# bernardo-torres/1d-spectral-optimal-transport

Hardware: AMD Instinct MI355X
Metric: sot_loss_evals_per_sec (higher is better)
Workload: dtype f32

## Files before the change

1d-spectral-optimal-transport_amd/csrc/sot_full_common.hpp:

```cpp
#pragma once
#include "sot_launch.hpp"

namespace sot {

#ifdef SOT_STAMPS
#define SOT_PH(sacc, i) do { if ((sacc) != nullptr) { __builtin_amdgcn_sched_barrier(0); const unsigned long long now_ = __builtin_readcyclecounter(); \
                              (sacc)[i] += now_ - (sacc)[15]; (sacc)[15] = now_; __builtin_amdgcn_sched_barrier(0); } } while (0)
#else
#define SOT_PH(sacc, i) do { } while (0)
#endif

template <int NSTEPS>
__device__ __forceinline__ float mass_column_nx(const float* part, int c)
{
    constexpr int NFULL = NSTEPS >> 4;
    constexpr int NREAD = NFULL + ((NSTEPS & 15) ? 1 : 0);
    float pre[NREAD];
#pragma unroll
    for (int h = 0; h < NREAD; ++h) pre[h] = part[(h << 5) + c];
    float a0 = 0.0f, a1 = 0.0f, a2 = 0.0f, a3 = 0.0f;
#pragma unroll
    for (int h = 0; h < NFULL; ++h) {
        a0 = pre[h];
        a1 += a0; a0 = 0.0f;
        if ((((h + 1) << 4) & (15 << 4)) == 0) {
            a2 += a1; a1 = 0.0f;
            if ((((h + 1) << 4) & (15 << 8)) == 0) { a3 += a2; a2 = 0.0f; }
        }
    }
    if (NSTEPS & 15) a0 = pre[NFULL];
    return ((a0 + a1) + a2) + a3;
}

__host__ __device__ constexpr int staged_index(int e, bool swz) { return swz ? (e ^ (((e >> 5) & 1) << 2)) : e; }

template <bool SQ, int N, bool SWZ>
__device__ __forceinline__ float mass_fold_nx(const float* raw, const float* colbuf)
{
    const float4* c4 = reinterpret_cast<const float4*>(colbuf);
    const float4 a0 = c4[0], a1 = c4[1], b0 = c4[2], b1 = c4[3], c0 = c4[4], c1 = c4[5], d0 = c4[6], d1 = c4[7];
    const float p0 = ((a0.x + b0.x) + c0.x) + d0.x, p1 = ((a0.y + b0.y) + c0.y) + d0.y;
    const float p2 = ((a0.z + b0.z) + c0.z) + d0.z, p3 = ((a0.w + b0.w) + c0.w) + d0.w;
    const float p4 = ((a1.x + b1.x) + c1.x) + d1.x, p5 = ((a1.y + b1.y) + c1.y) + d1.y;
    const float p6 = ((a1.z + b1.z) + c1.z) + d1.z, p7 = ((a1.w + b1.w) + c1.w) + d1.w;
    float fin = 0.0f;
#pragma unroll
    for (int k = (N >> 3) << 3; k < N; ++k) { const float w = raw[staged_index(k, SWZ)]; fin += SQ ? w * w : w; }
    fin += p0; fin += p1; fin += p2; fin += p3; fin += p4; fin += p5; fin += p6; fin += p7;
    return fin;
}

#define SOT_FULL_WALK_UNROLL 32

template <int NU, int NV>
__device__ __forceinline__ uint32_t merge_path_fixed32(uint32_t ub1, uint32_t vd1, int D)
{
    constexpr int TOPK = merge_steps_top(NU < NV ? NU : NV);
    const int lo = max(0, D - NV), hi = min(D, NU);
    uint32_t posb = ub1 + 4u * (uint32_t)lo;
    const uint32_t hib = ub1 + 4u * (uint32_t)hi;
#pragma unroll
    for (int k = TOPK; k >= -1; --k) {
        const uint32_t step4 = 4u * (uint32_t)(k >= 1 ? (1 << k) + 1 : (k == 0 ? 2 : 1));
        const uint32_t candb = posb + step4;
        const float u = lds_load(candb);
        const float v = lds_load(vd1 - candb);
        const int take = (int)(candb <= hib) & (int)(u <= v);
        posb = take ? candb : posb;
    }
    return posb;
}

template <int G, int CPT, int N>
__device__ __forceinline__ void fetch_row_dwords(const float* __restrict__ x, const float* __restrict__ y, int t, float (&rx)[CPT],
                                                 float (&ry)[CPT])
{
#pragma unroll
    for (int k = 0; k < CPT; ++k) {
        if (k * G < N) {
            const int e = t + k * G;
            const bool ok = ((k + 1) * G <= N) || (e < N);
            rx[k] = ok ? x[e] : 0.0f;
            ry[k] = ok ? y[e] : 0.0f;
        }
    }
}

typedef __amdgpu_buffer_rsrc_t RowBuffer;
__device__ __forceinline__ RowBuffer row_buffer(const float* row, int n)
{
    return __builtin_amdgcn_make_buffer_rsrc(const_cast<float*>(row), (short)0, n * 4, 0x00020000);
}
__device__ __forceinline__ float row_buffer_load(RowBuffer rb, int element)
{
    return __builtin_bit_cast(float, __builtin_amdgcn_raw_buffer_load_b32(rb, element * 4, 0, 0));
}
__device__ __forceinline__ void row_buffer_store(RowBuffer rb, int element, float v)
{
    __builtin_amdgcn_raw_buffer_store_b32(__builtin_bit_cast(unsigned int, v), rb, element * 4, 0, 0);
}

template <int G, int CPT>
__device__ __forceinline__ void fetch_row_dwords_rt(const float* __restrict__ x, const float* __restrict__ y, int t, int n, float (&rx)[CPT],
                                                    float (&ry)[CPT])
{
    const RowBuffer bx = row_buffer(x, n), by = row_buffer(y, n);
#pragma unroll
    for (int k = 0; k < CPT; ++k) {
        rx[k] = row_buffer_load(bx, t + k * G);
        ry[k] = row_buffer_load(by, t + k * G);
    }
}

template <int G, int CPT, int NX>
__device__ __forceinline__ void fetch_row(const float* __restrict__ x, const float* __restrict__ y, int t, int n, float (&rx)[CPT], float (&ry)[CPT]);

template <int G, int CPT>
__device__ __forceinline__ void fetch_full_row(const float* __restrict__ x, const float* __restrict__ y, int t, float (&rx)[CPT],
                                               float (&ry)[CPT])
{
    const float4* x4 = reinterpret_cast<const float4*>(x);
    const float4* y4 = reinterpret_cast<const float4*>(y);
#pragma unroll
    for (int k = 0; k < CPT / 4; ++k) {
        const float4 vx = x4[t + k * G], vy = y4[t + k * G];
        rx[4 * k] = vx.x; rx[4 * k + 1] = vx.y; rx[4 * k + 2] = vx.z; rx[4 * k + 3] = vx.w;
        ry[4 * k] = vy.x; ry[4 * k + 1] = vy.y; ry[4 * k + 2] = vy.z; ry[4 * k + 3] = vy.w;
    }
}

template <int G, int CPT>
__device__ __forceinline__ void fetch_row_columns(const float* __restrict__ x, const float* __restrict__ y, int t, float (&rx)[CPT], float (&ry)[CPT])
{
    static_assert(CPT == 8, "16 steps per task: two registers arrays of 8");
    const bool isy = t >= G / 2;
    const int task = isy ? t - G / 2 : t;
    const float* const src = (isy ? y : x) + ((task >> 5) << 9) + (task & 31);
#pragma unroll
    for (int k = 0; k < 8; ++k) { rx[k] = src[k << 5]; ry[k] = src[(8 + k) << 5]; }
}

template <int G, int CPT, int N>
struct ColumnsNX {
    static constexpr int NSTEPS = N >> 5, NCH = (NSTEPS + 15) >> 4, NT = 32 * NCH, CHUNK = NSTEPS < 16 ? NSTEPS : 16;
    static constexpr int TPT = (2 * NT) / G;
    static constexpr int NV = TPT * CHUNK;
    static constexpr int MIN_BINS = 1025;
    static constexpr bool OK = (2 * NT) % G == 0 && TPT >= 1 && NV + 1 <= 2 * CPT && (N & 7) == 1 && N >= MIN_BINS;
};
template <int CPT>
__device__ __forceinline__ float& column_slot(float (&rx)[CPT], float (&ry)[CPT], int j) { return j < CPT ? rx[j] : ry[j - CPT]; }

template <int G, int CPT, int N>
__device__ __forceinline__ void fetch_row_columns_nx(const float* __restrict__ x, const float* __restrict__ y, int t, float (&rx)[CPT], float (&ry)[CPT])
{
    using C = ColumnsNX<G, CPT, N>;
#pragma unroll
    for (int i = 0; i < C::TPT; ++i) {
        const int id = t + i * G;
        const bool isy = id >= C::NT;
        const int task = isy ? id - C::NT : id;
        const float* const src = (isy ? y : x) + ((task >> 5) << 9) + (task & 31);
#pragma unroll
        for (int k = 0; k < C::CHUNK; ++k) column_slot<CPT>(rx, ry, i * C::CHUNK + k) = src[k << 5];
    }
    float tail = 0.0f;
    if (t < 2) tail = (t ? y : x)[N - 1];
    column_slot<CPT>(rx, ry, C::NV) = tail;
}

template <int G, int CPT, int NX>
__device__ __forceinline__ void fetch_row(const float* __restrict__ x, const float* __restrict__ y, int t, int n, float (&rx)[CPT], float (&ry)[CPT])
{
    if constexpr (NX == 0) fetch_row_columns<G, CPT>(x, y, t, rx, ry);
    else if constexpr (NX > 0 && ColumnsNX<G, CPT, (NX > 0 ? NX : 129)>::OK) fetch_row_columns_nx<G, CPT, NX>(x, y, t, rx, ry);
    else if constexpr (NX == 0) fetch_full_row<G, CPT>(x, y, t, rx, ry);
    else if constexpr (NX > 0) fetch_row_dwords<G, CPT, NX>(x, y, t, rx, ry);
    else fetch_row_dwords_rt<G, CPT>(x, y, t, n, rx, ry);
}

struct FullLayout {
    int padcap;
    int nU, nV;
    int part;
    int colbuf;
    int wtot;
    int red;
    int grad;
    int goff;
    int rowf;
    int posf;
    int total;
};

template <int G, int CPT, int ROWS, int GRAD = 0, int NX = 0>
__host__ __device__ constexpr FullLayout full_layout()
{
    constexpr int CAP = G * CPT, N = NX > 0 ? NX : CAP, NW = G / kWave, NT = 32 * (((N >> 5) + 15) >> 4);
    FullLayout L{};
    L.padcap = align4(merge_steps(2 * N, G)) + 4;
    L.nU = L.padcap + CAP + 4;
    L.nV = CAP + 4;
    L.part = L.nU + L.nV;
    L.colbuf = L.part + 2 * NT;
    L.wtot = L.colbuf + 64;
    L.red = L.wtot + 4 * NW;
    L.grad = align4(L.red + NW + 4);
    L.goff = GRAD == 2 ? L.grad - L.nU : L.grad;
    L.rowf = GRAD == 2 ? L.grad + L.nV : GRAD ? L.grad + L.nU + L.nV : L.grad;
    L.posf = L.nU + L.nV;
    L.total = ROWS * L.rowf + L.posf;
    return L;
}

template <int G, int CPT, int ROWS, int GRAD, int NX = 0>
struct FullGeo {
    static_assert(ROWS >= 1 && ROWS <= 4, "row groups per workgroup");
    static constexpr int CAP = G * CPT;
    static constexpr bool RT = NX < 0;
    static constexpr int N = NX > 0 ? NX : CAP;
    static constexpr bool ALIGNED = (NX == 0);
    static constexpr int NSTEPS = N >> 5;
    static_assert(N <= CAP && N >= 64 && CPT >= 2 && CPT <= 17, "the row fits its geometry");
    static_assert(!ALIGNED || CPT == 8, "rows that fill their geometry: 8 contiguous elements (two 16-B halves) per thread");
    static constexpr bool SWZ = CPT == 8 && !RT;
    static_assert(NX <= 0 || CAP - N >= 1, "NX is for rows shorter than the capacity");
    static_assert(RT || NSTEPS < 16 || NSTEPS % 16 == 0, "every column is either one partial chunk or whole 16-step chunks");
    static_assert(RT || (N >> 3) == NSTEPS * 4, "no left-over 8-lane vectors (N mod 32 < 8)");
    static_assert(!SWZ || ((N >> 5) & 1) == 0 || (N & 7) == 0, "the scalar tail sits in an unswapped staging block");
    static_assert(((G >> 5) & 1) == 0, "the staging swizzle of element t + k*G must not depend on k");
    static constexpr int BLOCK = ROWS * G;
    static constexpr int NW = G / kWave;
    static constexpr int K = 2 * N;
    static constexpr int E = merge_steps(K, G);
    static constexpr int GA = (K + E - 1) / E;
    static constexpr int PAD = GA * E - K;
    static constexpr int NCH = (NSTEPS + 15) >> 4;
    static constexpr int CHUNK = NSTEPS < 16 ? NSTEPS : 16;
    static constexpr int NT = 32 * NCH;
    static constexpr FullLayout L = full_layout<G, CPT, ROWS, GRAD, NX>();
    static_assert(PAD + 1 <= L.padcap, "room for the virtual predecessor in front of the padding");
};

struct FullCtx {
    float* U; float* V; float* part; float* colbuf; double* wtot; float* red; float* Sv;
    const float* Uw;
    const float* PX; const float* PY;
    int rg, t, lane, wv;
    bool dn, x_ident, y_ident;
};

template <int G, int CPT, int ROWS, int GRAD, int NX = 0, bool RP = false>
__device__ __forceinline__ FullCtx full_setup(const FwdArgs& a, float* smem)
{
    using Geo = FullGeo<G, CPT, ROWS, GRAD, NX>;
    constexpr FullLayout L = Geo::L;
    constexpr int N = Geo::N, PAD = Geo::PAD;
    FullCtx c;
    const int tid = threadIdx.x;
    c.rg = __builtin_amdgcn_readfirstlane(tid / G);
    c.t = tid - c.rg * G;
    c.lane = tid & (kWave - 1);
    c.wv = __builtin_amdgcn_readfirstlane(c.t >> 6);
    c.dn = a.flags & SOT_FLAG_DONT_NORMALIZE;
    float* const base = smem + c.rg * L.rowf;
    c.U = base + L.padcap;
    c.V = base + L.nU;
    c.part = base + L.part;
    c.colbuf = base + L.colbuf;
    c.wtot = reinterpret_cast<double*>(base + L.wtot);
    c.red = base + L.red;
    c.Sv = c.red + Geo::NW;
    c.Uw = c.U - PAD;
    c.x_ident = true; c.y_ident = true;
    if (a.ident != nullptr) { c.x_ident = a.ident[0] != 0; c.y_ident = a.ident[1] != 0; }
    float* const PX = smem + ROWS * L.rowf + L.padcap;
    float* const PY = smem + ROWS * L.rowf + L.nU;
    c.PX = PX; c.PY = PY;
    const int nlast = (Geo::RT ? a.n : N) - 1;
    if (!RP) {
#pragma unroll
        for (int e = tid; e < N; e += Geo::BLOCK) {
            const int es = Geo::RT ? min(e, nlast) : e;
            PX[e] = a.xpos[es]; PY[e] = a.ypos[es];
        }
        if (tid < PAD) PX[tid - PAD] = a.xpos[0];
        if (tid == 0) {
            PX[N] = a.xpos[nlast];
            PY[N] = a.ypos[nlast];
        }
    }
    if (c.t < PAD) c.U[c.t - PAD] = 0.0f;
    for (int e = N + 1 + c.t; e < Geo::CAP; e += G) { c.U[e] = 0.0f; c.V[e] = 0.0f; }
    if (c.t == 0) {
        c.U[N] = INFINITY; c.V[N] = INFINITY;
        c.U[-PAD - 1] = -INFINITY; c.V[-1] = -INFINITY;
        if (Geo::RT) { c.U[N + 1] = 0.0f; c.V[N + 1] = 0.0f; }
    }
    return c;
}

template <int G, int CPT, int ROWS, int GRAD, bool SQ, int NX = 0, bool TO_LDS = true, bool RAW_OUT = (GRAD != 0)>
__device__ __forceinline__ void full_build_cdfs(const FwdArgs& a, const FullCtx& c, float (&rx)[CPT], float (&ry)[CPT],
                                                const float* nxt_x, const float* nxt_y, float (&wx)[CPT], float (&wy)[CPT],
                                                float& Sx, float& Sy, float (&cu)[CPT], float (&cv)[CPT], unsigned long long* sacc = nullptr,
                                                const int* psx = nullptr, const int* psy = nullptr)
{
    (void)sacc;
    using Geo = FullGeo<G, CPT, ROWS, GRAD, NX>;
    constexpr int N = Geo::N, NW = Geo::NW, NT = Geo::NT, CHUNK = Geo::CHUNK;
    constexpr bool ALIGNED = Geo::ALIGNED, RT = Geo::RT;
    float* const U = c.U; float* const V = c.V; float* const part = c.part; float* const colbuf = c.colbuf;
    double* const wtot = c.wtot; float* const Sv = c.Sv;
    const int t = c.t, lane = c.lane, wv = c.wv;
    const bool dn = c.dn, x_ident = c.x_ident, y_ident = c.y_ident;
    constexpr bool SWZ = Geo::SWZ;
    static_assert(G % 16 == 0, "whole 16-lane groups per row");
    const int q0s = SWZ ? (t ^ ((t >> 3) & 1)) : t;
    const int ownf = SWZ ? ((t >> 2) & 1) : 0;
    constexpr bool COLUMNS_NX = (NX > 0) && ColumnsNX<G, CPT, (NX > 0 ? NX : 129)>::OK;
    constexpr bool COLUMNS = ALIGNED || COLUMNS_NX;
    constexpr bool PRESQ = COLUMNS && SQ && !RAW_OUT;
    if constexpr (COLUMNS_NX) {
        using C = ColumnsNX<G, CPT, (NX > 0 ? NX : 129)>;
        static_assert(!COLUMNS_NX || (C::NT == NT && C::CHUNK == CHUNK && !SWZ), "the task layout of the chunk sums below");
#pragma unroll
        for (int i = 0; i < C::TPT; ++i) {
            const int id = t + i * G;
            const bool isy = id >= NT;
            const int task = isy ? id - NT : id;
            float* const dst = (isy ? V : U) + ((task >> 5) << 9) + (task & 31);
            float v[C::CHUNK];
#pragma unroll
            for (int k = 0; k < C::CHUNK; ++k) { const float w = column_slot<CPT>(rx, ry, i * C::CHUNK + k); v[k] = PRESQ ? w * w : w; }
#pragma unroll
            for (int k = 0; k < C::CHUNK; ++k) dst[k << 5] = v[k];
            if (!(isy && dn)) {
                float acc = 0.0f;
#pragma unroll
                for (int k = 0; k < C::CHUNK; ++k) acc += (SQ && !PRESQ) ? v[k] * v[k] : v[k];
                part[id] = acc;
            }
        }
        if (t < 2) { const float w = column_slot<CPT>(rx, ry, C::NV); (t ? V : U)[N - 1] = PRESQ ? w * w : w; }
    } else if constexpr (COLUMNS) {
        static_assert(2 * NT == G, "one (column, chunk) task per thread");
        const bool isy = t >= NT;
        const int task = isy ? t - NT : t;
        float* const dst = (isy ? V : U) + ((task >> 5) << 9) + (task & 31);
        float* const dsto = (isy ? V : U) + ((task >> 5) << 9) + ((task & 31) ^ (SWZ ? 4 : 0));
        float v[16];
#pragma unroll
        for (int k = 0; k < 8; ++k) { v[k] = PRESQ ? rx[k] * rx[k] : rx[k]; v[8 + k] = PRESQ ? ry[k] * ry[k] : ry[k]; }
#pragma unroll
        for (int k = 0; k < 16; ++k) ((k & 1) ? dsto : dst)[k << 5] = v[k];
        if (!(isy && dn)) {
            float acc = 0.0f;
#pragma unroll
            for (int k = 0; k < 16; ++k) acc += (SQ && !PRESQ) ? v[k] * v[k] : v[k];
            part[t] = acc;
        }
    } else if constexpr (ALIGNED) {
#pragma unroll
        for (int k = 0; k < CPT / 4; ++k) {
            reinterpret_cast<float4*>(U)[q0s + k * G] = make_float4(rx[4 * k], rx[4 * k + 1], rx[4 * k + 2], rx[4 * k + 3]);
            reinterpret_cast<float4*>(V)[q0s + k * G] = make_float4(ry[4 * k], ry[4 * k + 1], ry[4 * k + 2], ry[4 * k + 3]);
        }
    } else {
        const int es = SWZ ? (t ^ (((t >> 5) & 1) << 2)) : t;
#pragma unroll
        for (int k = 0; k < CPT; ++k) {
            if (RT || (k * G < N && (((k + 1) * G <= N) || (t + k * G < N)))) { U[es + k * G] = rx[k]; V[es + k * G] = ry[k]; }
        }
    }
    SOT_PH(sacc, 1);
    row_sync<NW>();
    SOT_PH(sacc, 2);

    const MassPlan mp = make_mass_plan(RT ? a.n : N);
    if constexpr (COLUMNS) {
    } else if constexpr (RT) {
        mass_chunk_sums<G, SQ>(U, part, mp, t);
        if (!dn) mass_chunk_sums<G, SQ>(V, part + NT, mp, t);
    } else {
#pragma unroll
    for (int id0 = 0; id0 < 2 * NT; id0 += G) {
        const int id = id0 + t;
        const bool isy = id >= NT;
        if (id < 2 * NT && !(isy && dn)) {
            const int task = isy ? id - NT : id;
            const float* src = (isy ? V : U) + ((task >> 5) << 9) + (task & 31);
            const float* srco = (isy ? V : U) + ((task >> 5) << 9) + ((task & 31) ^ (SWZ ? 4 : 0));
            float v[CHUNK];
#pragma unroll
            for (int s2 = 0; s2 < CHUNK; ++s2) { const float w = ((s2 & 1) ? srco : src)[s2 << 5]; v[s2] = SQ ? w * w : w; }
            float acc = 0.0f;
#pragma unroll
            for (int s2 = 0; s2 < CHUNK; ++s2) acc += v[s2];
            part[id] = acc;
        }
    }
    }
    SOT_PH(sacc, 3);
    if constexpr (!COLUMNS) row_sync<NW>();
    SOT_PH(sacc, 4);
    __builtin_amdgcn_s_setprio(kMassPrio);
    if (NW >= 2) {
        if (wv < 2 && !(wv == 1 && dn)) {
            const float* raw = wv ? V : U;
            float* cb = colbuf + 32 * wv;
            if (lane < 32) {
                if constexpr (RT) cb[lane] = mass_column<SQ>(raw, part + wv * NT, mp, lane);
                else cb[lane] = mass_column_nx<Geo::NSTEPS>(part + wv * NT, lane);
            }
            __builtin_amdgcn_fence(__ATOMIC_RELEASE, "wavefront");
            __builtin_amdgcn_wave_barrier();
            __builtin_amdgcn_fence(__ATOMIC_ACQUIRE, "wavefront");
            float S;
            if constexpr (RT) S = mass_fold<SQ>(raw, cb, mp.n);
            else S = mass_fold_nx<(SQ && !PRESQ), N, SWZ>(raw, cb);
            if (lane == 0) { Sv[wv] = S; Sv[2 + wv] = 1.0f / guard_mass(S); }
        }
    } else {
        const int half = lane >> 5, col = lane & 31;
        const bool use_y = half && !dn;
        float* cb = colbuf + 32 * half;
        if constexpr (RT) cb[col] = mass_column<SQ>(use_y ? V : U, part + (use_y ? NT : 0), mp, col);
        else cb[col] = mass_column_nx<Geo::NSTEPS>(part + (use_y ? NT : 0), col);
        __builtin_amdgcn_fence(__ATOMIC_RELEASE, "wavefront");
        __builtin_amdgcn_wave_barrier();
        __builtin_amdgcn_fence(__ATOMIC_ACQUIRE, "wavefront");
        float S;
        if constexpr (RT) S = mass_fold<SQ>(use_y ? V : U, cb, mp.n);
        else S = mass_fold_nx<(SQ && !PRESQ), N, SWZ>(use_y ? V : U, cb);
        if (col == 0) { Sv[half] = S; Sv[2 + half] = 1.0f / guard_mass(S); }
    }
    __builtin_amdgcn_s_setprio(0);
    const int e0 = t * CPT;
    const int h0 = e0 + 4 * ownf, h1 = e0 + 4 * (1 - ownf);
    if (x_ident) {
        if constexpr (CPT == 8) {
            const float4 v0 = *reinterpret_cast<const float4*>(U + h0), v1 = *reinterpret_cast<const float4*>(U + h1);
            wx[0] = v0.x; wx[1] = v0.y; wx[2] = v0.z; wx[3] = v0.w; wx[4] = v1.x; wx[5] = v1.y; wx[6] = v1.z; wx[7] = v1.w;
        } else {
#pragma unroll
            for (int k = 0; k < CPT; ++k) wx[k] = U[e0 + k];
        }
    } else if (psx != nullptr) {
#pragma unroll
        for (int k = 0; k < CPT; ++k) wx[k] = U[psx[k]];
    } else {
#pragma unroll
        for (int k = 0; k < CPT; ++k) {
            const int sx = (e0 + k < (RT ? a.n : N)) ? a.xperm[e0 + k] : N + 1;
            wx[k] = U[SWZ ? (sx ^ (((sx >> 5) & 1) << 2)) : sx];
        }
    }
    if (y_ident) {
        if constexpr (CPT == 8) {
            const float4 v0 = *reinterpret_cast<const float4*>(V + h0), v1 = *reinterpret_cast<const float4*>(V + h1);
            wy[0] = v0.x; wy[1] = v0.y; wy[2] = v0.z; wy[3] = v0.w; wy[4] = v1.x; wy[5] = v1.y; wy[6] = v1.z; wy[7] = v1.w;
        } else {
#pragma unroll
            for (int k = 0; k < CPT; ++k) wy[k] = V[e0 + k];
        }
    } else if (psy != nullptr) {
#pragma unroll
        for (int k = 0; k < CPT; ++k) wy[k] = V[psy[k]];
    } else {
#pragma unroll
        for (int k = 0; k < CPT; ++k) {
            const int sy = (e0 + k < (RT ? a.n : N)) ? a.yperm[e0 + k] : N + 1;
            wy[k] = V[SWZ ? (sy ^ (((sy >> 5) & 1) << 2)) : sy];
        }
    }
    if ((N < Geo::CAP || RT) && e0 + CPT > (RT ? a.n : N)) {
#pragma unroll
        for (int k = 0; k < CPT; ++k) {
            if (e0 + k >= (RT ? a.n : N)) { wx[k] = 0.0f; wy[k] = 0.0f; }
        }
    }
    SOT_PH(sacc, 5);
    row_sync<NW>();
    SOT_PH(sacc, 6);

    Sx = Sv[0]; Sy = dn ? Sx : Sv[1];
    const float rSx = Sv[2], rSy = dn ? rSx : Sv[3];
    const float Sxh = guard_mass(Sx), Syh = guard_mass(Sy);
    double px[CPT], py[CPT];
    double runx = 0.0, runy = 0.0;
    {
        float qx[CPT], qy[CPT];
        uint32_t risk = 0xFFFFFFFFu;
#pragma unroll
        for (int k = 0; k < CPT; ++k) {
            qx[k] = div_by_row_constant((SQ && !PRESQ) ? wx[k] * wx[k] : wx[k], Sxh, rSx, risk);
            qy[k] = div_by_row_constant((SQ && !PRESQ) ? wy[k] * wy[k] : wy[k], Syh, rSy, risk);
        }
        const bool slow = (risk < kFastDivMinBits) || !(Sxh <= 0x1p40f) || !(Syh <= 0x1p40f);
        if (__builtin_amdgcn_ballot_w64(slow) != 0ull) {
            asm volatile("; IEEE division fallback" ::: "memory");
#pragma unroll
            for (int k = 0; k < CPT; ++k) {
                qx[k] = ((SQ && !PRESQ) ? wx[k] * wx[k] : wx[k]) / Sxh;
                qy[k] = ((SQ && !PRESQ) ? wy[k] * wy[k] : wy[k]) / Syh;
            }
        }
#pragma unroll
        for (int k = 0; k < CPT; ++k) {
            runx += (double)qx[k]; runy += (double)qy[k];
            px[k] = runx; py[k] = runy;
        }
    }
    const double inx = wave_incl_scan(runx), iny = wave_incl_scan(runy);
    double exx = wave_shift_right1(inx), exy = wave_shift_right1(iny);
    if (NW > 1 && lane == kWave - 1) { wtot[wv] = inx; wtot[NW + wv] = iny; }
    SOT_PH(sacc, 7);
    row_sync<NW>();
    SOT_PH(sacc, 8);
    if constexpr (NW > 1) {
        double ox = 0.0, oy = 0.0;
        for (int w = 0; w < wv; ++w) { ox += wtot[w]; oy += wtot[NW + w]; }
        exx += ox; exy += oy;
    }
#pragma unroll
    for (int k = 0; k < CPT; ++k) { cu[k] = (float)(exx + px[k]); cv[k] = (float)(exy + py[k]); }
    if constexpr (TO_LDS) {
        if (CPT % 4 == 0 && (N == Geo::CAP || e0 + CPT <= N)) {
#pragma unroll
            for (int k = 0; k + 3 < CPT; k += 4) {
                *reinterpret_cast<float4*>(U + e0 + k) = make_float4(cu[k], cu[k + 1], cu[k + 2], cu[k + 3]);
                *reinterpret_cast<float4*>(V + e0 + k) = make_float4(cv[k], cv[k + 1], cv[k + 2], cv[k + 3]);
            }
        } else {
#pragma unroll
            for (int k = 0; k < CPT; ++k) {
                if (e0 + k < N) { U[e0 + k] = cu[k]; V[e0 + k] = cv[k]; }
            }
        }
    }
    if (nxt_x != nullptr) fetch_row<G, CPT, NX>(nxt_x, nxt_y, t, a.n, rx, ry);
    if constexpr (TO_LDS) row_sync<NW>();
}

template <int G, int CPT, int ROWS, int GRAD, int NX>
__device__ __forceinline__ void rowpos_row_setup(const FwdArgs& a, const FullCtx& c, int64_t rowc, int (&ix)[CPT], int (&iy)[CPT], int (&psx)[CPT], int (&psy)[CPT])
{
    using Geo = FullGeo<G, CPT, ROWS, GRAD, NX>;
    constexpr int N = Geo::N, NW = Geo::NW, PAD = Geo::PAD;
    static_assert(ROWS == 1 && NX == 0 && CPT == 8, "per-row positions: one row per workgroup, rows that fill the 8-element geometry");
    const int t = c.t;
    const uint16_t* const pr = a.perm_in + rowc * (2 * (int64_t)N);
    const float* const xp = a.xpos + rowc * a.xps;
    const float* const yp = a.ypos + rowc * a.yps;
    const uint4 qx = *reinterpret_cast<const uint4*>(pr + t * CPT), qy = *reinterpret_cast<const uint4*>(pr + N + t * CPT);
    float vx[CPT], vy[CPT];
#pragma unroll
    for (int k = 0; k < CPT; ++k) { vx[k] = xp[t + k * G]; vy[k] = yp[t + k * G]; }
    const uint32_t wqx[4] = {qx.x, qx.y, qx.z, qx.w}, wqy[4] = {qy.x, qy.y, qy.z, qy.w};
#pragma unroll
    for (int k = 0; k < CPT; ++k) {
        ix[k] = (int)((wqx[k >> 1] >> (16 * (k & 1))) & (uint32_t)(N - 1));
        iy[k] = (int)((wqy[k >> 1] >> (16 * (k & 1))) & (uint32_t)(N - 1));
        psx[k] = Geo::SWZ ? (ix[k] ^ (((ix[k] >> 5) & 1) << 2)) : ix[k];
        psy[k] = Geo::SWZ ? (iy[k] ^ (((iy[k] >> 5) & 1) << 2)) : iy[k];
    }
    float* const Um = c.U; float* const Vm = c.V;
#pragma unroll
    for (int k = 0; k < CPT; ++k) { Um[t + k * G] = vx[k]; Vm[t + k * G] = vy[k]; }
    row_sync<NW>();
    float gx[CPT], gy[CPT];
#pragma unroll
    for (int k = 0; k < CPT; ++k) { gx[k] = Um[ix[k]]; gy[k] = Vm[iy[k]]; }
    float* const PXw = const_cast<float*>(c.PX); float* const PYw = const_cast<float*>(c.PY);
    *reinterpret_cast<float4*>(PXw + t * CPT) = make_float4(gx[0], gx[1], gx[2], gx[3]);
    *reinterpret_cast<float4*>(PXw + t * CPT + 4) = make_float4(gx[4], gx[5], gx[6], gx[7]);
    *reinterpret_cast<float4*>(PYw + t * CPT) = make_float4(gy[0], gy[1], gy[2], gy[3]);
    *reinterpret_cast<float4*>(PYw + t * CPT + 4) = make_float4(gy[4], gy[5], gy[6], gy[7]);
    if (t < PAD) PXw[t - PAD] = gx[0];
    if (t == G - 1) { PXw[N] = gx[CPT - 1]; PYw[N] = gy[CPT - 1]; }
    row_sync<NW>();
}

}
```

1d-spectral-optimal-transport_amd/csrc/sot_full_fwd.hpp:

```cpp
#pragma once
#include "sot_full_common.hpp"

namespace sot {

constexpr int kFwd17MinWaves = 1;

constexpr int kFwd1025OneWaveRows = 6144;
constexpr int kRt1024OneWaveRows = 8192;

template <int E, int PM, bool LIM, uint32_t POFF4>
__device__ __forceinline__ float merge_walk_full(uint32_t ou, uint32_t ov, bool first, float p)
{
    float w = lds_load(ou), wp = lds_load(ou + POFF4);
    float r = lds_load(ov), rp = lds_load(ov + POFF4);
    float qprev = fmaxf(lds_load(ou - 4u), lds_load(ov - 4u));
    if (first) qprev = 0.0f;
    uint32_t pw = ou + 4u, pr = ov + 4u;
    float acc = 0.0f;
#pragma unroll SOT_FULL_WALK_UNROLL
    for (int s2 = 0; s2 < E; ++s2) {
        const bool c = w <= r;
        const float q = c ? w : r;
        const float cost = transport_cost<PM>(wp, rp, p);
        float delta = q - qprev;
        if (LIM && q > 1.0f) delta = 0.0f;
        acc = fmaf(delta, cost, acc);
        qprev = q;
        const uint32_t nx = c ? pw : pr;
        pr = c ? pr : pw;
        pw = nx + 4u;
        r = c ? r : w;
        rp = c ? rp : wp;
        w = lds_load(nx);
        wp = lds_load(nx + POFF4);
    }
    return acc;
}

template <int G, int CPT, int ROWS, int NX>
__device__ __forceinline__ void owner_perm_slots(const FwdArgs& a, const int* perm, int t, int (&ps)[CPT])
{
    using Geo = FullGeo<G, CPT, ROWS, false, NX>;
    constexpr int N = Geo::N;
    const int nreal = Geo::RT ? a.n : N;
#pragma unroll
    for (int k = 0; k < CPT; ++k) {
        const int sx = (t * CPT + k < nreal) ? perm[t * CPT + k] : N + 1;
        ps[k] = Geo::SWZ ? (sx ^ (((sx >> 5) & 1) << 2)) : sx;
    }
}

constexpr int kFwdMinWaves = 1;
constexpr int kRt512MinWaves = 4;

template <int G, int CPT, int ROWS, int PM, bool LIM, bool SQ, int NX = 0, bool RP = false>
__global__ __launch_bounds__(ROWS * G, (G == 512 && NX < 0) ? kRt512MinWaves : (CPT == 17) ? kFwd17MinWaves : kFwdMinWaves) void sot_forward_full_kernel(const FwdArgs a)
{
    static_assert(!RP || (ROWS == 1 && NX == 0 && CPT == 8), "per-row positions: one row per workgroup, rows that fill the 8-element geometry");
    using Geo = FullGeo<G, CPT, ROWS, false, NX>;
    constexpr FullLayout L = Geo::L;
    constexpr int N = Geo::N, NW = Geo::NW, E = Geo::E, GA = Geo::GA, PAD = Geo::PAD;
    extern __shared__ __attribute__((aligned(16))) float smem[];
    const int64_t row_step = (int64_t)gridDim.x * ROWS;
    int64_t row0 = (int64_t)blockIdx.x * ROWS;
    float rx[CPT], ry[CPT];
    FullCtx cm = full_setup<G, CPT, ROWS, false, NX, RP>(a, smem);
    if constexpr (RP) { cm.x_ident = false; cm.y_ident = false; }
    const FullCtx c = cm;
    if constexpr (NW == 1) __syncthreads();
    const int rg = c.rg, t = c.t, lane = c.lane, wv = c.wv;
    float* const V = c.V; float* const red = c.red;
    const float* const Uw = c.Uw;
    if (row0 < a.B) {
        const int64_t r = min(row0 + rg, a.B - 1);
        fetch_row<G, CPT, NX>(a.x + r * a.xs, a.y + r * a.ys, t, a.n, rx, ry);
    }

#ifdef SOT_STAMPS
    unsigned long long sbuf[16] = {};
    unsigned long long* const sacc = (threadIdx.x == 0 && blockIdx.x == gridDim.x / 2) ? sbuf : nullptr;
#else
    constexpr unsigned long long* sacc = nullptr;
#endif
    constexpr bool HOIST_PERM = CPT <= 9;
    int psx[HOIST_PERM ? CPT : 1] = {}, psy[HOIST_PERM ? CPT : 1] = {};
    if constexpr (HOIST_PERM && !RP) {
        if (!c.x_ident) owner_perm_slots<G, CPT, ROWS, NX>(a, a.xperm, t, psx);
        if (!c.y_ident) owner_perm_slots<G, CPT, ROWS, NX>(a, a.yperm, t, psy);
    }
    for (; row0 < a.B; row0 += row_step) {
        const int64_t row = row0 + rg;
        const bool valid = row < a.B;
        const bool more = row0 + row_step < a.B;
        const int64_t rn = min(row0 + row_step + rg, a.B - 1);
        float wx[CPT], wy[CPT], cu[CPT], cv[CPT];
        float Sx, Sy;
#ifdef SOT_STAMPS
        if (sacc != nullptr) sacc[15] = __builtin_readcyclecounter();
#endif
        if constexpr (RP) {
            int ix[CPT], iy[CPT];
            rowpos_row_setup<G, CPT, ROWS, false, NX>(a, c, min(row, a.B - 1), ix, iy, psx, psy);
        }
        full_build_cdfs<G, CPT, ROWS, false, SQ, NX>(a, c, rx, ry, more ? a.x + rn * a.xs : nullptr,
                                                     more ? a.y + rn * a.ys : nullptr, wx, wy, Sx, Sy, cu, cv, sacc, HOIST_PERM ? psx : nullptr,
                                                     HOIST_PERM ? psy : nullptr);
        SOT_PH(sacc, 9);

        float acc = 0.0f;
        __builtin_amdgcn_s_setprio(kWalkPrio);
        if (GA == G || t < GA) {
            constexpr int VOFF = L.nU - L.padcap + PAD;
            const int D0 = t * E;
            (void)VOFF;
            const uint32_t ub1 = lds_addr(Uw) - 4u;
            const uint32_t vd1 = lds_addr(V) + 4u * (uint32_t)D0 + ub1;
            const uint32_t pb = merge_path_fixed32<N + PAD, N>(ub1, vd1, D0);
            SOT_PH(sacc, 10);
            const uint32_t ou = pb + 4u;
            const uint32_t ov = vd1 - pb;
            constexpr uint32_t ROWB = 4u * (uint32_t)L.rowf;
            if (ROWS == 1 || rg == ROWS - 1) acc = merge_walk_full<E, PM, LIM, ROWB>(ou, ov, D0 == 0, a.p);
            else if (ROWS == 2 || rg == ROWS - 2) acc = merge_walk_full<E, PM, LIM, 2u * ROWB>(ou, ov, D0 == 0, a.p);
            else if (ROWS == 3 || rg == ROWS - 3) acc = merge_walk_full<E, PM, LIM, 3u * ROWB>(ou, ov, D0 == 0, a.p);
            else acc = merge_walk_full<E, PM, LIM, 4u * ROWB>(ou, ov, D0 == 0, a.p);
        }
        __builtin_amdgcn_s_setprio(0);
        SOT_PH(sacc, 11);
        acc = wave_sum(acc);
        if (NW == 1) {
            if (lane == 0 && valid && a.row_loss) store_row_loss(a.row_loss, row, acc, a.mt.counters != nullptr);
            row_sync<NW>();
        } else {
            if (lane == 0) red[wv] = acc;
            row_sync<NW>();
            if (t == 0 && valid && a.row_loss) {
                float tot = red[0];
#pragma unroll
                for (int w = 1; w < NW; ++w) tot += red[w];
                store_row_loss(a.row_loss, row, tot, a.mt.counters != nullptr);
            }
        }
        SOT_PH(sacc, 12);
#ifdef SOT_STAMPS
        if (sacc != nullptr) sacc[0] += 1;
#endif
    }
#ifdef SOT_STAMPS
    if (sacc != nullptr) { for (int i = 0; i < 16; ++i) g_stamps[i] = sacc[i]; }
#endif
    if (a.mt.counters != nullptr) batch_mean_tail<ROWS * G>(a.mt, a.row_loss, a.B, reinterpret_cast<double*>(smem));
}

constexpr int kAreaMinWaves = 1;
template <int G, int CPT, int ROWS, bool SQ, int NX = 0>
__global__ __launch_bounds__(ROWS * G, (CPT == 17) ? kFwd17MinWaves : kAreaMinWaves) void sot_area_full_kernel(const FwdArgs a)
{
    using Geo = FullGeo<G, CPT, ROWS, false, NX>;
    constexpr FullLayout L = Geo::L;
    constexpr int N = Geo::N, NW = Geo::NW;
    extern __shared__ __attribute__((aligned(16))) float smem[];
    const int64_t row_step = (int64_t)gridDim.x * ROWS;
    int64_t row0 = (int64_t)blockIdx.x * ROWS;
    const int tid = threadIdx.x;
    FullCtx c;
    c.rg = __builtin_amdgcn_readfirstlane(tid / G);
    c.t = tid - c.rg * G;
    c.lane = tid & (kWave - 1);
    c.wv = __builtin_amdgcn_readfirstlane(c.t >> 6);
    const int rg = c.rg, t = c.t, lane = c.lane, wv = c.wv;
    float rx[CPT], ry[CPT];
    if (row0 < a.B) {
        const int64_t r = min(row0 + rg, a.B - 1);
        fetch_row<G, CPT, NX>(a.x + r * a.xs, a.y + r * a.ys, t, a.n, rx, ry);
    }
    c.dn = a.flags & SOT_FLAG_DONT_NORMALIZE;
    float* const base = smem + rg * L.rowf;
    c.U = base + L.padcap; c.V = base + L.nU; c.part = base + L.part; c.colbuf = base + L.colbuf;
    c.wtot = reinterpret_cast<double*>(base + L.wtot);
    c.red = base + L.red; c.Sv = c.red + NW;
    c.Uw = c.U; c.PX = nullptr; c.PY = nullptr;
    c.x_ident = true; c.y_ident = true;
    if (a.ident != nullptr) { c.x_ident = a.ident[0] != 0; c.y_ident = a.ident[1] != 0; }
    float dx[CPT];
    {
        const int e0 = t * CPT;
        float pe[CPT + 1];
        const int nreal = Geo::RT ? a.n : N;
#pragma unroll
        for (int k = 0; k <= CPT; ++k) pe[k] = a.xpos[min(e0 + k, nreal - 1)];
#pragma unroll
        for (int k = 0; k < CPT; ++k) dx[k] = (e0 + k + 1 < nreal) ? pe[k + 1] - pe[k] : 0.0f;
    }
    float* const red = c.red;
#ifdef SOT_STAMPS
    unsigned long long sbuf[16] = {};
    unsigned long long* const sacc = (threadIdx.x == 0 && blockIdx.x == gridDim.x / 2) ? sbuf : nullptr;
#endif

    for (; row0 < a.B; row0 += row_step) {
        const int64_t row = row0 + rg;
        const bool valid = row < a.B;
        const bool more = row0 + row_step < a.B;
        const int64_t rn = min(row0 + row_step + rg, a.B - 1);
        float wx[CPT], wy[CPT], cu[CPT], cv[CPT];
        float Sx, Sy;
#ifdef SOT_STAMPS
        if (sacc != nullptr) sacc[15] = __builtin_readcyclecounter();
        full_build_cdfs<G, CPT, ROWS, false, SQ, NX, false>(a, c, rx, ry, more ? a.x + rn * a.xs : nullptr,
                                                            more ? a.y + rn * a.ys : nullptr, wx, wy, Sx, Sy, cu, cv, sacc);
        SOT_PH(sacc, 9);
#else
        full_build_cdfs<G, CPT, ROWS, false, SQ, NX, false>(a, c, rx, ry, more ? a.x + rn * a.xs : nullptr,
                                                            more ? a.y + rn * a.ys : nullptr, wx, wy, Sx, Sy, cu, cv);
#endif
        float acc = 0.0f;
#pragma unroll
        for (int k = 0; k < CPT; ++k) acc = fmaf(fabsf(cu[k] - cv[k]), dx[k], acc);
        acc = wave_sum(acc);
        if (NW == 1) {
            if (lane == 0 && valid && a.row_loss) store_row_loss(a.row_loss, row, acc, a.mt.counters != nullptr);
            row_sync<NW>();
        } else {
            if (lane == 0) red[wv] = acc;
            row_sync<NW>();
            if (t == 0 && valid && a.row_loss) {
                float tot = red[0];
#pragma unroll
                for (int w = 1; w < NW; ++w) tot += red[w];
                store_row_loss(a.row_loss, row, tot, a.mt.counters != nullptr);
            }
        }
#ifdef SOT_STAMPS
        SOT_PH(sacc, 10);
        if (sacc != nullptr) sacc[0] += 1;
#endif
    }
#ifdef SOT_STAMPS
    if (sacc != nullptr) { for (int i = 0; i < 16; ++i) g_stamps[i] = sacc[i]; }
#endif
    if (a.mt.counters != nullptr) batch_mean_tail<ROWS * G>(a.mt, a.row_loss, a.B, reinterpret_cast<double*>(smem));
}

__device__ __forceinline__ double half_incl_scan(double v)
{
    v += dpp_f64_shr<kRowShr1>(v);
    v += dpp_f64_shr<kRowShr2>(v);
    v += dpp_f64_shr<kRowShr4>(v);
    v += dpp_f64_shr<kRowShr8>(v);
    v += dpp_f64<kRowBcast15, 0xA>(v);
    return v;
}
__device__ __forceinline__ double half_shift_right1(double v, int l)
{
    const double s = dpp_f64<kWaveShr1>(v);
    return l == 0 ? 0.0 : s;
}
__device__ __forceinline__ float half_sum(float v, int h)
{
    v += dpp_f32<kRowShr1>(v);
    v += dpp_f32<kRowShr2>(v);
    v += dpp_f32<kRowShr4>(v);
    v += dpp_f32<kRowShr8>(v);
    v += dpp_f32<kRowBcast15, 0xA>(v);
    const float t0 = __int_as_float(__builtin_amdgcn_readlane(__float_as_int(v), 31));
    const float t1 = __int_as_float(__builtin_amdgcn_readlane(__float_as_int(v), 63));
    return h ? t1 : t0;
}

template <int CPT, int N>
__device__ __forceinline__ void half_fetch(const float* __restrict__ x, const float* __restrict__ y, int l, float (&rx)[CPT], float (&ry)[CPT])
{
    constexpr int NK = (N + 31) >> 5;
#pragma unroll
    for (int k = 0; k < CPT; ++k) {
        rx[k] = 0.0f; ry[k] = 0.0f;
        if (k < NK) {
            const int e = l + 32 * k;
            if ((k + 1) * 32 <= N || e < N) { rx[k] = x[e]; ry[k] = y[e]; }
        }
    }
}

template <int CPT, bool SQ, int N>
__device__ __forceinline__ void half_stage(float* U, float* V, float* colbuf, int l, const float (&rx)[CPT], const float (&ry)[CPT])
{
    constexpr int NSTEPS = N >> 5, NK = (N + 31) >> 5;
    float ax = 0.0f, ay = 0.0f;
#pragma unroll
    for (int k = 0; k < NK; ++k) {
        const int e = l + 32 * k;
        if ((k + 1) * 32 <= N || e < N) { U[e] = rx[k]; V[e] = ry[k]; }
        if (k < NSTEPS) { ax += SQ ? rx[k] * rx[k] : rx[k]; ay += SQ ? ry[k] * ry[k] : ry[k]; }
    }
    colbuf[l] = ax; colbuf[32 + l] = ay;
}

template <int CPT, bool SQ, int N>
__device__ __forceinline__ void half_cdfs(const FwdArgs& a, const float* U, const float* V, const float* colbuf, int l, bool dn, bool x_ident,
                                          bool y_ident, float (&cu)[CPT], float (&cv)[CPT])
{
    const int e0 = l * CPT;
    const float Sx = mass_fold_nx<SQ, N, false>(U, colbuf);
    const float Sy = dn ? Sx : mass_fold_nx<SQ, N, false>(V, colbuf + 32);
    float wx[CPT], wy[CPT];
#pragma unroll
    for (int k = 0; k < CPT; ++k) {
        const bool in = e0 + k < N;
        const int sx = in ? (x_ident ? e0 + k : a.xperm[e0 + k]) : 0;
        const int sy = in ? (y_ident ? e0 + k : a.yperm[e0 + k]) : 0;
        wx[k] = in ? U[sx] : 0.0f;
        wy[k] = in ? V[sy] : 0.0f;
    }
    const float Sxh = guard_mass(Sx), Syh = guard_mass(Sy);
    const float rSx = 1.0f / Sxh, rSy = 1.0f / Syh;
    double px[CPT], py[CPT];
    double runx = 0.0, runy = 0.0;
    {
        float qx[CPT], qy[CPT];
        uint32_t risk = 0xFFFFFFFFu;
#pragma unroll
        for (int k = 0; k < CPT; ++k) {
            qx[k] = div_by_row_constant(SQ ? wx[k] * wx[k] : wx[k], Sxh, rSx, risk);
            qy[k] = div_by_row_constant(SQ ? wy[k] * wy[k] : wy[k], Syh, rSy, risk);
        }
        const bool slow = (risk < kFastDivMinBits) || !(Sxh <= 0x1p40f) || !(Syh <= 0x1p40f);
        if (__builtin_amdgcn_ballot_w64(slow) != 0ull) {
#pragma unroll
            for (int k = 0; k < CPT; ++k) {
                qx[k] = (SQ ? wx[k] * wx[k] : wx[k]) / Sxh;
                qy[k] = (SQ ? wy[k] * wy[k] : wy[k]) / Syh;
            }
        }
#pragma unroll
        for (int k = 0; k < CPT; ++k) {
            runx += (double)qx[k]; runy += (double)qy[k];
            px[k] = runx; py[k] = runy;
        }
    }
    const double exx = half_shift_right1(half_incl_scan(runx), l), exy = half_shift_right1(half_incl_scan(runy), l);
#pragma unroll
    for (int k = 0; k < CPT; ++k) { cu[k] = (float)(exx + px[k]); cv[k] = (float)(exy + py[k]); }
}

template <int CPT, int ROWS, bool SQ, int N>
__global__ __launch_bounds__(ROWS * 32) void sot_area_half_kernel(const FwdArgs a)
{
    constexpr int CAP = 32 * CPT, NSTEPS = N >> 5, NK = (N + 31) >> 5;
    static_assert(ROWS % 2 == 0 && NK <= CPT && N <= CAP && NSTEPS >= 1 && NSTEPS < 16, "two half-wave rows per wave; one partial ATen chunk per column");
    static_assert((N >> 3) == NSTEPS * 4, "no left-over 8-lane vectors (N mod 32 < 8)");
    constexpr int ROWF = 2 * (CAP + 4) + 64 + 8;
    extern __shared__ __attribute__((aligned(16))) float smem[];
    const int tid = threadIdx.x, lane = tid & (kWave - 1), l = lane & 31, h = lane >> 5, rs = tid >> 5;
    float* const U = smem + rs * ROWF;
    float* const V = U + CAP + 4;
    float* const colbuf = V + CAP + 4;
    const bool dn = a.flags & SOT_FLAG_DONT_NORMALIZE;
    bool x_ident = true, y_ident = true;
    if (a.ident != nullptr) { x_ident = a.ident[0] != 0; y_ident = a.ident[1] != 0; }
    const int64_t row_step = (int64_t)gridDim.x * ROWS;
    int64_t row0 = (int64_t)blockIdx.x * ROWS;
    const int e0 = l * CPT;
    float dx[CPT];
    {
        float pe[CPT + 1];
#pragma unroll
        for (int k = 0; k <= CPT; ++k) pe[k] = a.xpos[min(e0 + k, N - 1)];
#pragma unroll
        for (int k = 0; k < CPT; ++k) dx[k] = (e0 + k + 1 < N) ? pe[k + 1] - pe[k] : 0.0f;
    }
    float rx[CPT], ry[CPT];
    if (row0 < a.B) { const int64_t r = min(row0 + rs, a.B - 1); half_fetch<CPT, N>(a.x + r * a.xs, a.y + r * a.ys, l, rx, ry); }

    for (; row0 < a.B; row0 += row_step) {
        const int64_t row = row0 + rs;
        const bool valid = row < a.B;
        half_stage<CPT, SQ, N>(U, V, colbuf, l, rx, ry);
        if (row0 + row_step < a.B) { const int64_t r = min(row0 + row_step + rs, a.B - 1); half_fetch<CPT, N>(a.x + r * a.xs, a.y + r * a.ys, l, rx, ry); }
        row_sync<1>();
        float cu[CPT], cv[CPT];
        half_cdfs<CPT, SQ, N>(a, U, V, colbuf, l, dn, x_ident, y_ident, cu, cv);
        float acc = 0.0f;
#pragma unroll
        for (int k = 0; k < CPT; ++k) acc = fmaf(fabsf(cu[k] - cv[k]), dx[k], acc);
        acc = half_sum(acc, h);
        if (l == 0 && valid && a.row_loss) store_row_loss(a.row_loss, row, acc, a.mt.counters != nullptr);
        row_sync<1>();
    }
    if (a.mt.counters != nullptr) batch_mean_tail<ROWS * 32>(a.mt, a.row_loss, a.B, reinterpret_cast<double*>(smem));
}

template <int CPT, int ROWS, int PM, bool LIM, bool SQ, int N>
struct HalfRowGeo {
    static constexpr int CAP = 32 * CPT, K = 2 * N, E = merge_steps(K, 32), GA = (K + E - 1) / E, PAD = GA * E - K;
    static constexpr int PADCAP = align4(E) + 4, NU = PADCAP + CAP + 4, NV = CAP + 4;
    static constexpr int POFF = NU + NV + 64;
    static constexpr int ROWF = POFF + NU + NV;
    static_assert(GA <= 32 && PAD + 1 <= PADCAP, "every lane walks at most one segment; room for the virtual predecessor");
};

template <int CPT, int ROWS, int PM, bool LIM, bool SQ, int N>
__global__ __launch_bounds__(ROWS * 32) void sot_forward_half_kernel(const FwdArgs a)
{
    using H = HalfRowGeo<CPT, ROWS, PM, LIM, SQ, N>;
    constexpr int CAP = H::CAP, NSTEPS = N >> 5, NK = (N + 31) >> 5, E = H::E, GA = H::GA, PAD = H::PAD;
    static_assert(ROWS % 2 == 0 && NK <= CPT && N <= CAP && NSTEPS >= 1 && NSTEPS < 16 && (N >> 3) == NSTEPS * 4, "see sot_area_half_kernel");
    extern __shared__ __attribute__((aligned(16))) float smem[];
    const int tid = threadIdx.x, lane = tid & (kWave - 1), l = lane & 31, h = lane >> 5, rs = tid >> 5;
    float* const base = smem + rs * H::ROWF;
    float* const U = base + H::PADCAP;
    float* const V = base + H::NU;
    float* const colbuf = base + H::NU + H::NV;
    float* const PX = U + H::POFF;
    float* const PY = V + H::POFF;
    const bool dn = a.flags & SOT_FLAG_DONT_NORMALIZE;
    bool x_ident = true, y_ident = true;
    if (a.ident != nullptr) { x_ident = a.ident[0] != 0; y_ident = a.ident[1] != 0; }
    for (int e = l; e < N; e += 32) { PX[e] = a.xpos[e]; PY[e] = a.ypos[e]; }
    if (l < PAD) { PX[l - PAD] = a.xpos[0]; U[l - PAD] = 0.0f; }
    if (l == 0) {
        PX[N] = a.xpos[N - 1]; PY[N] = a.ypos[N - 1];
        U[N] = INFINITY; V[N] = INFINITY;
        U[-PAD - 1] = -INFINITY; V[-1] = -INFINITY;
    }
    const int64_t row_step = (int64_t)gridDim.x * ROWS;
    int64_t row0 = (int64_t)blockIdx.x * ROWS;
    const int e0 = l * CPT;
    float rx[CPT], ry[CPT];
    if (row0 < a.B) { const int64_t r = min(row0 + rs, a.B - 1); half_fetch<CPT, N>(a.x + r * a.xs, a.y + r * a.ys, l, rx, ry); }
    row_sync<1>();

    for (; row0 < a.B; row0 += row_step) {
        const int64_t row = row0 + rs;
        const bool valid = row < a.B;
        half_stage<CPT, SQ, N>(U, V, colbuf, l, rx, ry);
        row_sync<1>();
        float cu[CPT], cv[CPT];
        half_cdfs<CPT, SQ, N>(a, U, V, colbuf, l, dn, x_ident, y_ident, cu, cv);
        row_sync<1>();
#pragma unroll
        for (int k = 0; k < CPT; ++k) {
            if (e0 + k < N) { U[e0 + k] = cu[k]; V[e0 + k] = cv[k]; }
        }
        if (row0 + row_step < a.B) { const int64_t r = min(row0 + row_step + rs, a.B - 1); half_fetch<CPT, N>(a.x + r * a.xs, a.y + r * a.ys, l, rx, ry); }
        row_sync<1>();
        float acc = 0.0f;
        if (GA == 32 || l < GA) {
            const int D0 = l * E;
            const uint32_t ub1 = lds_addr(U - PAD) - 4u;
            const uint32_t vd1 = lds_addr(V) + 4u * (uint32_t)D0 + ub1;
            const uint32_t pb = merge_path_fixed32<N + PAD, N>(ub1, vd1, D0);
            acc = merge_walk_full<E, PM, LIM, 4u * (uint32_t)H::POFF>(pb + 4u, vd1 - pb, D0 == 0, a.p);
        }
        acc = half_sum(acc, h);
        if (l == 0 && valid && a.row_loss) store_row_loss(a.row_loss, row, acc, a.mt.counters != nullptr);
        row_sync<1>();
    }
    if (a.mt.counters != nullptr) batch_mean_tail<ROWS * 32>(a.mt, a.row_loss, a.B, reinterpret_cast<double*>(smem));
}

template <int G, int CPT, int ROWS, bool SQ, int NX>
static hipError_t launch_area_full(const FwdArgs& a, hipStream_t s)
{
    constexpr FullLayout L = full_layout<G, CPT, ROWS, false, NX>();
    return launch_persistent<sot_area_full_kernel<G, CPT, ROWS, SQ, NX>, true>(a, sizeof(float) * (size_t)ROWS * (size_t)L.rowf, (a.B + ROWS - 1) / ROWS,
                                                                               ROWS * G, s);
}

template <int G, int CPT, int ROWS, int NX = 0>
static hipError_t dispatch_area_full_g(const FwdArgs& a, hipStream_t s)
{
    return (a.flags & SOT_FLAG_SQUARE) ? launch_area_full<G, CPT, ROWS, true, NX>(a, s) : launch_area_full<G, CPT, ROWS, false, NX>(a, s);
}

template <int CPT, int ROWS, bool SQ, int N>
static hipError_t launch_area_half(const FwdArgs& a, hipStream_t s)
{
    constexpr size_t lds = sizeof(float) * (size_t)ROWS * (2 * (32 * CPT + 4) + 64 + 8);
    return launch_persistent<sot_area_half_kernel<CPT, ROWS, SQ, N>, true>(a, lds, (a.B + ROWS - 1) / ROWS, ROWS * 32, s);
}

template <int CPT, int ROWS, int N>
static hipError_t dispatch_area_half(const FwdArgs& a, hipStream_t s)
{
    return (a.flags & SOT_FLAG_SQUARE) ? launch_area_half<CPT, ROWS, true, N>(a, s) : launch_area_half<CPT, ROWS, false, N>(a, s);
}

template <int G, int CPT, int ROWS, int PM, bool LIM, bool SQ, int NX, bool RP = false>
static hipError_t launch_forward_full(const FwdArgs& a, hipStream_t s)
{
    constexpr FullLayout L = full_layout<G, CPT, ROWS, false, NX>();
    return launch_persistent<sot_forward_full_kernel<G, CPT, ROWS, PM, LIM, SQ, NX, RP>, true>(a, sizeof(float) * (size_t)L.total, (a.B + ROWS - 1) / ROWS,
                                                                                               ROWS * G, s);
}

template <int G, int CPT, int ROWS, int NX = 0>
static hipError_t dispatch_forward_full_g(int pm, const FwdArgs& a, hipStream_t s)
{
    static_assert(sizeof(float) * (size_t)full_layout<G, CPT, ROWS, false, NX>().total <= kLdsLimit, "workgroup fits one CU's LDS");
    return with_mode(pm, a.flags, [&](auto md) { using M = decltype(md); return launch_forward_full<G, CPT, ROWS, M::PM, M::LIM, M::SQ, NX>(a, s); });
}

template <int G>
static hipError_t dispatch_forward_full_rowpos_g(int pm, const FwdArgs& a, hipStream_t s)
{
    return with_mode(pm, a.flags, [&](auto md) { using M = decltype(md); return launch_forward_full<G, 8, 1, M::PM, M::LIM, M::SQ, 0, true>(a, s); });
}

template <int CPT, int ROWS, int PM, bool LIM, bool SQ, int N>
static hipError_t launch_forward_half(const FwdArgs& a, hipStream_t s)
{
    constexpr size_t lds = sizeof(float) * (size_t)ROWS * HalfRowGeo<CPT, ROWS, PM, LIM, SQ, N>::ROWF;
    return launch_persistent<sot_forward_half_kernel<CPT, ROWS, PM, LIM, SQ, N>, true>(a, lds, (a.B + ROWS - 1) / ROWS, ROWS * 32, s);
}

template <int CPT, int ROWS, int N>
static hipError_t dispatch_forward_half(int pm, const FwdArgs& a, hipStream_t s)
{
    return with_mode(pm, a.flags, [&](auto md) { using M = decltype(md); return launch_forward_half<CPT, ROWS, M::PM, M::LIM, M::SQ, N>(a, s); });
}

}
```

Before: 249.8 million.

## Add specialized plain row loop deferring loss reduction past next row's first barrier

```diff
diff --git a/1d-spectral-optimal-transport_amd/csrc/sot_full_common.hpp b/1d-spectral-optimal-transport_amd/csrc/sot_full_common.hpp
--- a/1d-spectral-optimal-transport_amd/csrc/sot_full_common.hpp
+++ b/1d-spectral-optimal-transport_amd/csrc/sot_full_common.hpp
@@ -300,11 +300,16 @@
     return c;
 }
 
-template <int G, int CPT, int ROWS, int GRAD, bool SQ, int NX = 0, bool TO_LDS = true, bool RAW_OUT = (GRAD != 0)>
+constexpr int kPrefixSelectMaxWaves = 4;
+
+struct NoRowHook { __device__ __forceinline__ void operator()() const {} };
+
+template <int G, int CPT, int ROWS, int GRAD, bool SQ, int NX = 0, bool TO_LDS = true, bool RAW_OUT = (GRAD != 0), bool PLAIN = false,
+          class AfterB1 = NoRowHook>
 __device__ __forceinline__ void full_build_cdfs(const FwdArgs& a, const FullCtx& c, float (&rx)[CPT], float (&ry)[CPT],
                                                 const float* nxt_x, const float* nxt_y, float (&wx)[CPT], float (&wy)[CPT],
                                                 float& Sx, float& Sy, float (&cu)[CPT], float (&cv)[CPT], unsigned long long* sacc = nullptr,
-                                                const int* psx = nullptr, const int* psy = nullptr)
+                                                const int* psx = nullptr, const int* psy = nullptr, AfterB1 after_b1 = AfterB1{})
 {
     (void)sacc;
     using Geo = FullGeo<G, CPT, ROWS, GRAD, NX>;
@@ -313,7 +318,7 @@
     float* const U = c.U; float* const V = c.V; float* const part = c.part; float* const colbuf = c.colbuf;
     double* const wtot = c.wtot; float* const Sv = c.Sv;
     const int t = c.t, lane = c.lane, wv = c.wv;
-    const bool dn = c.dn, x_ident = c.x_ident, y_ident = c.y_ident;
+    const bool dn = PLAIN ? false : c.dn, x_ident = PLAIN ? true : c.x_ident, y_ident = PLAIN ? true : c.y_ident;
     constexpr bool SWZ = Geo::SWZ;
     static_assert(G % 16 == 0, "whole 16-lane groups per row");
     const int q0s = SWZ ? (t ^ ((t >> 3) & 1)) : t;
@@ -376,6 +381,7 @@
     SOT_PH(sacc, 1);
     row_sync<NW>();
     SOT_PH(sacc, 2);
+    after_b1();
 
     const MassPlan mp = make_mass_plan(RT ? a.n : N);
     if constexpr (COLUMNS) {
@@ -518,9 +524,20 @@
     SOT_PH(sacc, 7);
     row_sync<NW>();
     SOT_PH(sacc, 8);
-    if constexpr (NW > 1) {
+    if constexpr (NW > 1 && (NW > kPrefixSelectMaxWaves || GRAD != 0)) {
         double ox = 0.0, oy = 0.0;
         for (int w = 0; w < wv; ++w) { ox += wtot[w]; oy += wtot[NW + w]; }
+        exx += ox; exy += oy;
+    } else if constexpr (NW > 1) {
+        double tx[NW - 1], ty[NW - 1];
+#pragma unroll
+        for (int w = 0; w < NW - 1; ++w) { tx[w] = wtot[w]; ty[w] = wtot[NW + w]; }
+        double ox = 0.0, oy = 0.0;
+#pragma unroll
+        for (int w = 0; w < NW - 1; ++w) {
+            const double sx = ox + tx[w], sy = oy + ty[w];
+            ox = (w < wv) ? sx : ox; oy = (w < wv) ? sy : oy;
+        }
         exx += ox; exy += oy;
     }
 #pragma unroll
diff --git a/1d-spectral-optimal-transport_amd/csrc/sot_full_fwd.hpp b/1d-spectral-optimal-transport_amd/csrc/sot_full_fwd.hpp
--- a/1d-spectral-optimal-transport_amd/csrc/sot_full_fwd.hpp
+++ b/1d-spectral-optimal-transport_amd/csrc/sot_full_fwd.hpp
@@ -153,6 +153,68 @@
 }
 
 constexpr int kAreaMinWaves = 1;
+
+template <int G, int CPT, int ROWS, int NX>
+constexpr bool kAreaPlainLoop = (G == 256 && CPT == 8 && ROWS == 1 && NX == 0);
+
+template <int G, int CPT, int ROWS, bool SQ, int NX>
+__device__ __forceinline__ void area_rows_plain(const FwdArgs& a, const FullCtx& c, float (&rx)[CPT], float (&ry)[CPT], const float (&dx)[CPT],
+                                                int64_t row0, int64_t row_step, unsigned long long* sacc)
+{
+    (void)sacc;
+    constexpr int NW = FullGeo<G, CPT, ROWS, false, NX>::NW;
+    const int rg = c.rg, t = c.t, lane = c.lane, wv = c.wv;
+    float* const red = c.red;
+    float* const row_loss = a.row_loss;
+    int64_t pending = -1;
+    const auto store_pending = [&] {
+        if (NW > 1 && t == G - kWave && pending >= 0) {
+            float tot = red[0];
+#pragma unroll
+            for (int w = 1; w < NW; ++w) tot += red[w];
+            row_loss[pending] = tot;
+        }
+    };
+    if (row0 >= a.B) return;
+    for (;;) {
+        const int64_t row = row0 + rg;
+        const bool valid = ROWS == 1 || row < a.B;
+        const int64_t next0 = row0 + row_step;
+        const bool more = next0 < a.B;
+        const int64_t rn = min(next0 + rg, a.B - 1);
+        float wx[CPT], wy[CPT], cu[CPT], cv[CPT];
+        float Sx, Sy;
+#ifdef SOT_STAMPS
+        if (sacc != nullptr) sacc[15] = __builtin_readcyclecounter();
+#endif
+        full_build_cdfs<G, CPT, ROWS, false, SQ, NX, false, false, true>(a, c, rx, ry, more ? a.x + rn * a.xs : nullptr,
+                                                                         more ? a.y + rn * a.ys : nullptr, wx, wy, Sx, Sy, cu, cv, sacc,
+                                                                         nullptr, nullptr, store_pending);
+        SOT_PH(sacc, 9);
+        float acc = 0.0f;
+#pragma unroll
+        for (int k = 0; k < CPT; ++k) acc = fmaf(fabsf(cu[k] - cv[k]), dx[k], acc);
+        acc = wave_sum(acc);
+        if (NW == 1) {
+            if (lane == 0 && valid) row_loss[row] = acc;
+            row_sync<NW>();
+        } else {
+            if (lane == 0) red[wv] = acc;
+            pending = valid ? row : -1;
+        }
+#ifdef SOT_STAMPS
+        SOT_PH(sacc, 10);
+        if (sacc != nullptr) sacc[0] += 1;
+#endif
+        if (!more) break;
+        row0 = next0;
+    }
+    if constexpr (NW > 1) {
+        row_sync<NW>();
+        store_pending();
+    }
+}
+
 template <int G, int CPT, int ROWS, bool SQ, int NX = 0>
 __global__ __launch_bounds__(ROWS * G, (CPT == 17) ? kFwd17MinWaves : kAreaMinWaves) void sot_area_full_kernel(const FwdArgs a)
 {
@@ -196,8 +258,16 @@
 #ifdef SOT_STAMPS
     unsigned long long sbuf[16] = {};
     unsigned long long* const sacc = (threadIdx.x == 0 && blockIdx.x == gridDim.x / 2) ? sbuf : nullptr;
-#endif
-
+#else
+    constexpr unsigned long long* sacc = nullptr;
+#endif
+
+    constexpr bool PLAIN_LOOP = kAreaPlainLoop<G, CPT, ROWS, NX>;
+    bool plain = false;
+    if constexpr (PLAIN_LOOP) plain = c.x_ident && c.y_ident && !c.dn && a.row_loss != nullptr && a.mt.counters == nullptr;
+    if (plain) {
+        if constexpr (PLAIN_LOOP) area_rows_plain<G, CPT, ROWS, SQ, NX>(a, c, rx, ry, dx, row0, row_step, sacc);
+    } else {
     for (; row0 < a.B; row0 += row_step) {
         const int64_t row = row0 + rg;
         const bool valid = row < a.B;
@@ -236,10 +306,11 @@
         if (sacc != nullptr) sacc[0] += 1;
 #endif
     }
+    if (a.mt.counters != nullptr) batch_mean_tail<ROWS * G>(a.mt, a.row_loss, a.B, reinterpret_cast<double*>(smem));
+    }
 #ifdef SOT_STAMPS
     if (sacc != nullptr) { for (int i = 0; i < 16; ++i) g_stamps[i] = sacc[i]; }
 #endif
-    if (a.mt.counters != nullptr) batch_mean_tail<ROWS * G>(a.mt, a.row_loss, a.B, reinterpret_cast<double*>(smem));
 }
 
 __device__ __forceinline__ double half_incl_scan(double v)
```

Measured after the change: 258.3 million, median of 6. 1.03x the previous value.
